# jamtrott/spmv-cache-trace

Measured on AMD Instinct MI355X. Metric: spmv_csr_gflops, higher is better.
Workload: dtype f64

## Files before the change

### spmv-cache-trace_amd/csrc/csr_runs.hpp

```cpp
#pragma once

#include "csr_wavetile.hpp"

namespace spmv {

constexpr int kRunChunkRows = 128;
constexpr int kRunWaves = 4;
constexpr int kRunLen = 5;
constexpr int kRunSlot = kRunLen * 128;

struct RunPattern {
    int rel[kRunLen];
};

__device__ __forceinline__ int4 scalar_load_i4(const int4 * p)
{
    typedef const v4i __attribute__((address_space(4))) * const_ptr;
    const v4i v = *reinterpret_cast<const_ptr>(reinterpret_cast<uintptr_t>(p));
    return make_int4(v[0], v[1], v[2], v[3]);
}

template <bool NT>
__device__ __forceinline__ void run_values_lds(const unsigned (&lds)[kRunLen], const double * ak, const unsigned (&o)[kRunLen])
{
    unsigned keep;
#define SPMV_RUN_DMA5(NTS)                                                                                                     \
    "s_nop 4\n\ts_mov_b32 %0, m0\n\t"                                                                                          \
    "s_mov_b32 m0, %1\n\ts_nop 0\n\tglobal_load_lds_dwordx4 %6, %11" NTS "\n\t"                                                \
    "s_mov_b32 m0, %2\n\ts_nop 0\n\tglobal_load_lds_dwordx4 %7, %11" NTS "\n\t"                                                \
    "s_mov_b32 m0, %3\n\ts_nop 0\n\tglobal_load_lds_dwordx4 %8, %11" NTS "\n\t"                                                \
    "s_mov_b32 m0, %4\n\ts_nop 0\n\tglobal_load_lds_dwordx4 %9, %11" NTS "\n\t"                                                \
    "s_mov_b32 m0, %5\n\ts_nop 0\n\tglobal_load_lds_dwordx4 %10, %11" NTS "\n\t"                                               \
    "s_mov_b32 m0, %0"
    if (NT)
        asm volatile(SPMV_RUN_DMA5(" nt") : "=&s"(keep) : "s"(lds[0]), "s"(lds[1]), "s"(lds[2]), "s"(lds[3]), "s"(lds[4]), "v"(o[0]),
                     "v"(o[1]), "v"(o[2]), "v"(o[3]), "v"(o[4]), "s"(ak) : "memory");
    else
        asm volatile(SPMV_RUN_DMA5("") : "=&s"(keep) : "s"(lds[0]), "s"(lds[1]), "s"(lds[2]), "s"(lds[3]), "s"(lds[4]), "v"(o[0]),
                     "v"(o[1]), "v"(o[2]), "v"(o[3]), "v"(o[4]), "s"(ak) : "memory");
#undef SPMV_RUN_DMA5
}

#define SPMV_RUN_ISSUE(LAST)                                                                                                   \
    "s_nop 4\n\t"                                                                                                              \
    "global_load_dwordx4 %0, %7, %8 nt\n\t"                                                                                    \
    "global_load_dwordx4 %1, %9, %14\n\t"                                                                                      \
    "global_load_dwordx4 %2, %10, %14\n\t"                                                                                     \
    "global_load_dwordx4 %3, %11, %14\n\t"                                                                                     \
    "global_load_dwordx4 %4, %12, %14\n\t"                                                                                     \
    "global_load_dwordx4 %5, %13, %14\n\t" LAST " %6, %15, %16\n\t"                                                            \
    "s_waitcnt vmcnt(0)"
__device__ __forceinline__ void run_issue_full(v2d_a8 & yv, v2d_a8 (&xv)[kRunLen], double & last, unsigned yo, const double * yb,
                                               const unsigned (&xo)[kRunLen], const double * x, unsigned lo, const double * ak)
{
    asm volatile(SPMV_RUN_ISSUE("global_load_dwordx2")
                 : "=&v"(yv), "=&v"(xv[0]), "=&v"(xv[1]), "=&v"(xv[2]), "=&v"(xv[3]), "=&v"(xv[4]), "=&v"(last)
                 : "v"(yo), "s"(yb), "v"(xo[0]), "v"(xo[1]), "v"(xo[2]), "v"(xo[3]), "v"(xo[4]), "s"(x), "v"(lo), "s"(ak)
                 : "memory");
}
__device__ __forceinline__ void run_issue_masked(v2d_a8 & yv, v2d_a8 (&xv)[kRunLen], unsigned & m2, unsigned yo, const double * yb,
                                                 const unsigned (&xo)[kRunLen], const double * x, unsigned mo, const uint8_t * mk)
{
    asm volatile(SPMV_RUN_ISSUE("global_load_ushort")
                 : "=&v"(yv), "=&v"(xv[0]), "=&v"(xv[1]), "=&v"(xv[2]), "=&v"(xv[3]), "=&v"(xv[4]), "=&v"(m2)
                 : "v"(yo), "s"(yb), "v"(xo[0]), "v"(xo[1]), "v"(xo[2]), "v"(xo[3]), "v"(xo[4]), "s"(x), "v"(mo), "s"(mk)
                 : "memory");
}
#undef SPMV_RUN_ISSUE

template <bool DENSE, bool NT>
__global__ __launch_bounds__(256) void csr_runs_kernel(int nchunks, int rows, int cols, const int4 * __restrict__ chunks,
                                                       const uint8_t * __restrict__ masks, RunPattern pat, const double * __restrict__ a,
                                                       const double * __restrict__ x, const double * y_in, double * y)
{
    __shared__ __attribute__((aligned(16))) double slots[kRunWaves][kRunSlot];
    const int wave = __builtin_amdgcn_readfirstlane((int) threadIdx.x >> 6);
    const int lane = (int) __lane_id();
    const int c = (int) blockIdx.x * kRunWaves + wave;
    asm volatile("" ::"s"(nchunks), "s"(rows), "s"(cols), "s"(chunks), "s"(masks), "s"(pat.rel[0]), "s"(pat.rel[1]), "s"(pat.rel[2]),
                 "s"(pat.rel[3]), "s"(pat.rel[4]), "s"(a), "s"(x), "s"(y_in), "s"(y));
    if (c >= nchunks)
        return;
    const double * slot = slots[wave];
    const unsigned lds = __builtin_amdgcn_readfirstlane((unsigned) reinterpret_cast<uintptr_t>((const __attribute__((address_space(3))) double *) slot));
    const int4 d = scalar_load_i4(chunks + c);
    const int row0 = DENSE ? c * kRunChunkRows : d.x;
    const int n = DENSE ? min(kRunChunkRows, rows - row0) : (d.z & 0xFF);
    const int e0 = d.y, entries = d.z >> 8, mslot = d.w;
    const int base = min(2 * lane, n - 2);
    const int kb = e0 & ~1, lead = e0 & 1;
    const int lastpair = ((e0 + entries - 1) & ~1) - kb;
    unsigned ldsi[kRunLen], vo[kRunLen];
#pragma unroll
    for (int i = 0; i < kRunLen; ++i) {
        ldsi[i] = lds + 1024u * i;
        vo[i] = 8u * (unsigned) min(128 * i + 2 * lane, lastpair);
    }
    int cx[kRunLen];
    unsigned xo[kRunLen];
#pragma unroll
    for (int p = 0; p < kRunLen; ++p) {
        cx[p] = row0 + base + pat.rel[p];
        xo[p] = 8u * (unsigned) min(max(cx[p], 0), cols - 2);
    }
    const double * ak = a + kb;
    run_values_lds<NT>(ldsi, ak, vo);
    v2d_a8 yv, xl[kRunLen];
    double zA = 0.0, zB = 0.0;
    if (mslot < 0) {
        double last;
        run_issue_full(yv, xl, last, 8u * (unsigned) base, y_in + row0, xo, x, 8u * (unsigned) (lead + entries - 1), ak);
        const double * v = slot + lead + base * kRunLen;
        const double vlast = base == n - 2 ? last : slot[min(lead + base * kRunLen + 2 * kRunLen - 1, kRunSlot - 1)];
#pragma unroll
        for (int p = 0; p < kRunLen; ++p) {
            zA += v[p] * xl[p].x;
            zB += (p == kRunLen - 1 ? vlast : v[kRunLen + p]) * xl[p].y;
        }
    } else {
        unsigned m2;
        run_issue_masked(yv, xl, m2, 8u * (unsigned) base, y_in + row0, xo, x, 2u * (unsigned) lane, masks + (size_t) mslot * kRunChunkRows);
        v2d_a8 xv[kRunLen];
#pragma unroll
        for (int p = 0; p < kRunLen; ++p)
            xv[p] = v2d_a8{cx[p] > cols - 2 ? xl[p].y : xl[p].x, cx[p] < 0 ? xl[p].x : xl[p].y};
        const unsigned m0 = m2 & 0xFFu, m1 = (m2 >> 8) & 0xFFu;
        const int cnt = __builtin_popcount(m0) + __builtin_popcount(m1);
        const int before = wave_inclusive_scan(cnt) - cnt;
        const bool own_pair = 2 * lane <= n - 2;
        const unsigned mA = own_pair ? m0 : 0u, mB = own_pair ? m1 : m0;
        int kA = lead + before, kB = lead + before + (own_pair ? __builtin_popcount(m0) : 0);
        double vA[kRunLen], vB[kRunLen];
#pragma unroll
        for (int p = 0; p < kRunLen; ++p) {
            vA[p] = slot[min(kA, kRunSlot - 1)];
            vB[p] = slot[min(kB, kRunSlot - 1)];
            kA += (mA >> p) & 1u;
            kB += (mB >> p) & 1u;
        }
        asm volatile("" : "+v"(vA[0]), "+v"(vA[1]), "+v"(vA[2]), "+v"(vA[3]), "+v"(vA[4]), "+v"(vB[0]), "+v"(vB[1]), "+v"(vB[2]), "+v"(vB[3]),
                     "+v"(vB[4]));
#pragma unroll
        for (int p = 0; p < kRunLen; ++p) {
            if ((mA >> p) & 1u)
                zA += vA[p] * xv[p].x;
            if ((mB >> p) & 1u)
                zB += vB[p] * xv[p].y;
        }
    }
    if (2 * lane <= n - 2) {
        const v2d_a8 out = {yv.x + zA, yv.y + zB};
        __builtin_nontemporal_store(out, reinterpret_cast<v2d_a8 *>(y + row0 + base));
    } else if (2 * lane == n - 1) {
        __builtin_nontemporal_store(yv.y + zB, y + row0 + base + 1);
    }
}

}
```

### spmv-cache-trace_amd/csrc/internal.hpp

```cpp
#pragma once

#include "spmv_hip_plan.h"
#include "spmv_hip_symmetric.h"
#include "spmv_hip_multivec.h"
#include "spmv_hip_transpose.h"
#include "spmv_hip_f32values.h"
#include "spmv_hip_compact.h"

#include <hip/hip_runtime.h>
#include <rccl/rccl.h>

#include <atomic>
#include <cstdint>
#include <string>
#include <vector>

#include "spmv_kernels.hpp"
#include "csr_segwin.hpp"

namespace spmvi {

int fail(int code, const char * what);
int fail_hip(hipError_t e, const char * call);
int check_csr_row_ptr(int32_t rows, int32_t cols, const int32_t * row_ptr);
// ... 47 lines not shown
    int long_blocks = 0;
    int32_t * d_blk_row = nullptr;
    int4 * d_tiles = nullptr;
    int ntiles = 0;
    int tile = 0;
    uint16_t * d_col16 = nullptr;
    const int32_t * compressed_from = nullptr;
    int narrow_tiles = 0;
    int shifted_tiles = 0;
    int xwin_tiles = 0;
    int longest_tile_row = 0;
    int spread_tiles = 0;
    spmv_hip_plan * inner = nullptr;
    int32_t * d_vrow_ptr = nullptr;
    int32_t * d_pcol = nullptr;
    double * d_pval = nullptr;
    const int32_t * panels_from_col = nullptr;
    const double * panels_from_val = nullptr;
    spmv::PanelInfo pinfo{};
    int panel_blocks = 0;
    int2 * d_blocks = nullptr;
    int nblocks16 = 0;
    int blockwin_tiles = 0;
    int32_t * d_rest_tiles = nullptr;
    int nrest_tiles = 0;
    int4 * d_run_chunks = nullptr;
    uint8_t * d_run_masks = nullptr;
    int32_t * d_run_rest = nullptr;
    int nrun_chunks = 0, nrun_rest = 0, run_len = 0, run_tiles = 0, run_masked_chunks = 0;
    long long run_entries = 0;
    spmv::RunPattern run_pattern{};
    bool run_dense = false;
    bool run_nt = false;
    int32_t * d_group_tiles = nullptr, * d_group_rest = nullptr;
    int ngroup_tiles = 0, ngroup_rest = 0;
    spmv::SegWinBlock * d_segblocks = nullptr;
    int nsegblocks = 0, seg_tiles_per_block = 0, segwin_tiles = 0, segwin_slots = 0;
    int32_t * d_patterns = nullptr;
    int npatterns = 0;
    int uniform_tiles = 0;
    int split_rows = 0;
    bool balanced = false;
    int32_t * d_colh = nullptr;
    int32_t * d_hub_column = nullptr;
    double * d_hubx = nullptr;
    int nhubs = 0, hub_threshold = 0;
    long long hub_entries = 0;
    int multi_window_tiles = 0;
    int block_hint = 0;
    int block_offset = 0;
    bool block_skewed = false;
    int hints_tried = 0;
    bool hint_from_bits = false;
    int colshare_tiles = 0;
    long long colshare_entries = 0;
    int block_candidate = 0;
    const uint32_t * group_bits = nullptr;
    int block_cuts = 0;
    int break_rows = 0;
    int block_tiles = 0;
    long long block_entries = 0;
    int stencil_mask_tiles = 0;
    long long stencil_mask_entries = 0;
    int masked_block_tiles = 0;
    long long masked_block_entries = 0;
    size_t meta_bytes = 0;
// ... 112 lines not shown
```

### spmv-cache-trace_amd/csrc/launch.hip

```cpp
#include "internal.hpp"
#ifdef SPMV_HIP_EXPERIMENTS
#include "csr_pipe.hpp"
#include <cstdlib>
#endif

#include <algorithm>

using namespace spmvi;

namespace {

template <int LPR>
void launch_vector(const spmv_hip_plan * pl, const int32_t * p, const int32_t * j, const double * a,
                   const double * x, double * y, hipStream_t s)
{
    hipLaunchKernelGGL((spmv::csr_vector_kernel<LPR, kBlock>), dim3(pl->workgroups), dim3(kBlock), 0, s,
                       pl->rows, p, j, a, x, y);
}

}

extern "C" {

int spmv_hip_csr_spmv(const spmv_hip_plan * pl, const int32_t * p, const int32_t * j,
                      const double * a, const double * x, double * y, void * stream)
{
    return spmv_hip_csr_spmv_out(pl, p, j, a, x, y, y, stream);
}

static int csr_spmv_launch(const spmv_hip_plan * pl, const int32_t * p, const int32_t * j, const double * a,
                           const double * x, const double * y_in, double * y, void * stream, const spmv::PeerY * peers, int * fused);

int spmv_hip_csr_spmv_out(const spmv_hip_plan * pl, const int32_t * p, const int32_t * j, const double * a,
                          const double * x, const double * y_in, double * y, void * stream)
{
    return csr_spmv_launch(pl, p, j, a, x, y_in, y, stream, nullptr, nullptr);
}

int spmv_hip_peer_push(const double * d_src, double * const * d_dst, int ndst, int64_t n, void * stream);

int spmv_hip_csr_spmv_out_peers(const spmv_hip_plan * pl, const int32_t * p, const int32_t * j, const double * a,
                                const double * x, const double * y_in, double * y, double * const * peer_y, int npeers,
                                int * fused_out, void * stream)
// ... 148 lines not shown
                                       pl->d_col16, a, x, y_in, y, pl->cols);
                    HIP_TRY(hipGetLastError());
                    return SPMV_HIP_OK;
                }
            }
#endif
            const int4 * vi_tiles = pl->d_tiles_vi ? pl->d_tiles_vi : pl->d_tiles;
            const int vi_ntiles = pl->d_tiles_vi ? pl->ntiles_vi : pl->ntiles;
            const unsigned vi_groups = (unsigned) ((vi_ntiles + 3) / 4);
            const bool all_blockwin = c16 && (pl->d_blocks || pl->d_segblocks) && pl->blockwin_tiles == pl->ntiles;
            const bool rest_forwards = peers && c16 && x32 && pl->d_segblocks && pl->split_rows == 0 && pl->tile == 512 && !xcd
                && (pl->blockwin_tiles == pl->ntiles || (pl->d_rest_tiles && pl->nrest_tiles > 0));
            if (all_blockwin) {
            } else if (rest_forwards) {
                hipLaunchKernelGGL((spmv::csr_wavetile_kernel<512, true, true, false, 0, 0, false, false, true, true>), dim3((unsigned) ((pl->nrest_tiles + 3) / 4)),
                                   dim3(256), 0, s, pl->nrest_tiles, pl->d_tiles, p, j, pl->d_col16, a, x, y_in, y, pl->nnz, pl->cols, exact, pl->d_patterns,
                                   spmv::PanelInfo{}, (const uint8_t *) nullptr, (const double *) nullptr, 0, *peers, pl->d_rest_tiles);
            } else if (c16 && (pl->d_blocks || pl->d_segblocks) && pl->d_rest_tiles && pl->nrest_tiles > 0 && pl->tile == 512 && !xcd) {
                const dim3 grid((unsigned) ((pl->nrest_tiles + 3) / 4));
                if (x32)
                    hipLaunchKernelGGL((spmv::csr_wavetile_kernel<512, true, true, false, 0, 0, false, false, false, true>), grid, dim3(256), 0, s,
                                       pl->nrest_tiles, pl->d_tiles, p, j, pl->d_col16, a, x, y_in, y, pl->nnz, pl->cols, exact, pl->d_patterns,
                                       spmv::PanelInfo{}, (const uint8_t *) nullptr, (const double *) nullptr, 0, spmv::PeerY{}, pl->d_rest_tiles);
                else
                    hipLaunchKernelGGL((spmv::csr_wavetile_kernel<512, true, false, false, 0, 0, false, false, false, true>), grid, dim3(256), 0, s,
                                       pl->nrest_tiles, pl->d_tiles, p, j, pl->d_col16, a, x, y_in, y, pl->nnz, pl->cols, exact, pl->d_patterns,
                                       spmv::PanelInfo{}, (const uint8_t *) nullptr, (const double *) nullptr, 0, spmv::PeerY{}, pl->d_rest_tiles);
            } else if (pl->d_run_chunks && pl->run_len == 5 && c16 && x32 && !xcd && !peers && !pl->d_group_tiles && !(pl->nvalues > 0 && pl->values_from == a)
                       && spmvi::aligned16(a)
#ifdef SPMV_HIP_EXPERIMENTS
                       && !abl
#endif
            ) {
                const dim3 grid((unsigned) ((pl->nrun_chunks + spmv::kRunWaves - 1) / spmv::kRunWaves));
                auto runs = pl->run_dense ? (pl->run_nt ? spmv::csr_runs_kernel<true, true> : spmv::csr_runs_kernel<true, false>)
                                          : (pl->run_nt ? spmv::csr_runs_kernel<false, true> : spmv::csr_runs_kernel<false, false>);
                hipLaunchKernelGGL(runs, grid, dim3(256), 0, s, pl->nrun_chunks, pl->rows, pl->cols, pl->d_run_chunks, pl->d_run_masks,
                                   pl->run_pattern, a, x, y_in, y);
                if (pl->nrun_rest > 0)
                    hipLaunchKernelGGL((spmv::csr_wavetile_kernel<512, true, true, false, 0, 0, false, false, false, true>), dim3((unsigned) ((pl->nrun_rest + 3) / 4)),
                                       dim3(256), 0, s, pl->nrun_rest, pl->d_tiles, p, j, pl->d_col16, a, x, y_in, y, pl->nnz, pl->cols, exact, pl->d_patterns,
                                       spmv::PanelInfo{}, (const uint8_t *) nullptr, (const double *) nullptr, 0, spmv::PeerY{}, pl->d_run_rest);
            } else
#ifdef SPMV_HIP_EXPERIMENTS
            if (pl->d_group_tiles && c16 && x32 && !xcd && !exact_order && pl->tile == 512 && (!peers || pl->split_rows == 0)) {
                const dim3 grid((unsigned) ((pl->ngroup_tiles + 3) / 4)), rest((unsigned) ((pl->ngroup_rest + 3) / 4));
                if (peers) {
                    hipLaunchKernelGGL((spmv::csr_rowgroup_kernel<true>), grid, dim3(256), 0, s, pl->ngroup_tiles, pl->d_group_tiles, pl->d_tiles, a, x, y_in,
                                       y, pl->cols, pl->d_patterns, *peers);
                    if (pl->ngroup_rest > 0)
                        hipLaunchKernelGGL((spmv::csr_wavetile_kernel<512, true, true, false, 0, 256, false, false, true, true>), rest, dim3(256), 0, s,
                                           pl->ngroup_rest, pl->d_tiles, p, j, pl->d_col16, a, x, y_in, y, pl->nnz, pl->cols, exact, pl->d_patterns,
                                           spmv::PanelInfo{}, (const uint8_t *) nullptr, (const double *) nullptr, 0, *peers, pl->d_group_rest);
                    *fused = 1;
                } else {
                    hipLaunchKernelGGL((spmv::csr_rowgroup_kernel<false>), grid, dim3(256), 0, s, pl->ngroup_tiles, pl->d_group_tiles, pl->d_tiles, a, x, y_in,
                                       y, pl->cols, pl->d_patterns);
                    if (pl->ngroup_rest > 0)
                        hipLaunchKernelGGL((spmv::csr_wavetile_kernel<512, true, true, false, 0, 256, false, false, false, true>), rest, dim3(256), 0, s,
                                           pl->ngroup_rest, pl->d_tiles, p, j, pl->d_col16, a, x, y_in, y, pl->nnz, pl->cols, exact, pl->d_patterns,
                                           spmv::PanelInfo{}, (const uint8_t *) nullptr, (const double *) nullptr, 0, spmv::PeerY{}, pl->d_group_rest);
                }
            } else
#endif
            if (!(pl->flags & SPMV_HIP_FLAG_NO_X_WINDOW) && (!exact_order || pl->longest_tile_row <= 32) && c16 && x32
                && pl->tile == 512 && !xcd && 2 * (long long) pl->xwin_tiles > pl->ntiles
                && !(pl->nvalues > 0 && pl->values_from == a) ) {
                if (peers && pl->split_rows == 0 && !pl->d_blocks && !pl->d_segblocks) {
                    hipLaunchKernelGGL((spmv::csr_wavetile_kernel<512, true, true, false, 0, 256, false, false, true>), dim3(pl->workgroups), dim3(256), 0, s,
                                       pl->ntiles, pl->d_tiles, p, j, pl->d_col16, a, x, y_in, y, pl->nnz, pl->cols, exact, pl->d_patterns, spmv::PanelInfo{},
                                       (const uint8_t *) nullptr, (const double *) nullptr, 0, *peers);
// ... 202 lines not shown
```

### spmv-cache-trace_amd/csrc/plan_csr.hip

```cpp
#include "internal.hpp"

#include <algorithm>
#include <cstdlib>
#include <cstring>
#include <new>
#include <system_error>
#include <thread>
#include <unordered_map>
#include <utility>

using namespace spmvi;

namespace {

constexpr size_t kStripedInts = (size_t) spmv::kCountStripes * spmv::kCountWidth;

template <typename T>
hipError_t read_striped(const T * d_counters, T * out, int n, hipStream_t s)
{
    T host[kStripedInts];
    hipError_t e = hipMemcpyAsync(host, d_counters, sizeof(host), hipMemcpyDeviceToHost, s);
    if (e == hipSuccess)
        e = hipStreamSynchronize(s);
    for (int i = 0; i < n; ++i) {
// ... 86 lines not shown
}

int verify_plan(const spmv_hip_plan * pl, const int32_t * d_column_index, hipStream_t s)
{
    if (!pl->d_col16 || pl->compressed_from != d_column_index)
        return SPMV_HIP_OK;
    unsigned long long sum = 0;
    int rc = device_column_checksum(d_column_index, pl->nnz, &sum, s);
    if (rc != SPMV_HIP_OK)
        return rc;
    if (sum != pl->column_checksum)
        return fail(SPMV_HIP_ERR_STATE, "the column array at this address is not the one the plan was compressed from "
                                        "(contents changed): make a new plan");
    return SPMV_HIP_OK;
}

static __global__ void run_gather_u16(const uint16_t * __restrict__ j16, const int32_t * __restrict__ idx, uint16_t * __restrict__ out, int n)
{
    const int i = (int) (blockIdx.x * blockDim.x + threadIdx.x);
    if (i < n)
        out[i] = j16[idx[i]];
}

void drop_stencil_runs(spmv_hip_plan * pl)
{
    for (void * q : {(void *) pl->d_run_chunks, (void *) pl->d_run_rest, (void *) pl->d_run_masks})
        if (q)
            (void) hipFree(q);
    pl->d_run_chunks = nullptr;
    pl->d_run_rest = nullptr;
    pl->d_run_masks = nullptr;
    pl->nrun_chunks = pl->nrun_rest = pl->run_len = pl->run_tiles = pl->run_masked_chunks = 0;
    pl->run_entries = 0;
    pl->run_dense = pl->run_nt = false;
}

static int build_stencil_runs(spmv_hip_plan * pl, const std::vector<int4> & d, bool compressed)
{
    drop_stencil_runs(pl);
    const bool exact_order = (pl->flags & SPMV_HIP_FLAG_EXACT_ORDER) != 0;
    const bool xwin_launch = !(pl->flags & SPMV_HIP_FLAG_NO_X_WINDOW) && (!exact_order || pl->longest_tile_row <= 32)
        && 2 * (long long) pl->xwin_tiles > pl->ntiles;
    if ((pl->flags & (SPMV_HIP_FLAG_NO_STENCIL_RUNS | SPMV_HIP_FLAG_XCD_REMAP)) || !compressed || pl->nvalues > 0 || pl->balanced
        || pl->inner || pl->d_blocks || pl->d_segblocks || pl->tile != 512 || pl->npatterns == 0 || pl->cols >= (1 << 29) || xwin_launch
        || pl->algorithm != SPMV_HIP_CSR_WAVETILE || pl->ntiles == 0 || pl->cols < 2)
        return SPMV_HIP_OK;
    bool align = true, masked = true, early = false, nt = true;
#ifdef SPMV_HIP_EXPERIMENTS
    if (const char * v = std::getenv("SPMV_HIP_RUNS_ALIGN")) align = std::atoi(v) != 0;
    if (const char * v = std::getenv("SPMV_HIP_RUNS_MASKED")) masked = std::atoi(v) != 0;
    if (const char * v = std::getenv("SPMV_HIP_RUNS_EARLY")) early = std::atoi(v) != 0;
    if (const char * v = std::getenv("SPMV_HIP_RUNS_NT")) nt = std::atoi(v) != 0;
#endif
    constexpr int L = spmv::kRunLen;
    const int ntiles = pl->ntiles;
    auto values_len = [&](int w) -> int {
        const int4 t = d[(size_t) w];
        const int meta = t.z;
        const int k0 = t.y, k1 = d[(size_t) w + 1].y;
        const int need = spmv::kTileMetaFast | spmv::kTileMetaShifted | spmv::kTileMetaUniform | spmv::kTileMetaPattern;
        if ((t.x & spmv::kTileFlagPartial) || k1 <= k0 || (meta & need) != need || ((meta >> spmv::kTileMetaLanesShift) & 7) != 0
            || (meta & (spmv::kTileMetaBlockWin | spmv::kTileMetaBlock3)) || spmv::is_masked_stencil_tile(meta) || k1 - (k0 & ~3) > 512)
            return 0;
        return meta & 0xFFFF;
    };
    auto narrow_tile = [&](int w) -> bool {
        const int4 t = d[(size_t) w];
        const int meta = t.z;
        const int k0 = t.y, k1 = d[(size_t) w + 1].y;
        const int need = spmv::kTileMetaFast | spmv::kTileMetaNarrow | spmv::kTileMetaUniform;
        const int nrows = (d[(size_t) w + 1].x & ~spmv::kTileFlagPartial) - t.x;
        return !(t.x & spmv::kTileFlagPartial) && k1 > k0 && (meta & need) == need && ((meta >> spmv::kTileMetaLanesShift) & 7) == 0
            && !(meta & (spmv::kTileMetaShifted | spmv::kTileMetaPattern | spmv::kTileMetaBlockWin | spmv::kTileMetaBlock3))
            && (meta & 0xFFFF) >= 1 && (meta & 0xFFFF) <= L && nrows >= 1 && nrows <= spmv::kRunChunkRows
            && (long long) nrows * (meta & 0xFFFF) == (long long) (k1 - k0) && k1 - (k0 & ~3) <= 512;
    };
    auto masked_tile = [&](int w) -> bool {
        const int4 t = d[(size_t) w];
        return !(t.x & spmv::kTileFlagPartial) && d[(size_t) w + 1].y > t.y && (t.z & spmv::kTileMetaFast) && spmv::is_masked_stencil_tile(t.z)
            && !(t.z & (spmv::kTileMetaBlockWin | spmv::kTileMetaBlock3));
    };
    std::vector<long long> per_pattern((size_t) pl->npatterns, 0);
    for (int w = 0; w < ntiles; ++w)
        if (values_len(w) == L && d[(size_t) w].w >= 0 && d[(size_t) w].w < pl->npatterns)
            per_pattern[(size_t) d[(size_t) w].w] += (long long) d[(size_t) w + 1].y - d[(size_t) w].y;
// ... 167 lines not shown
            c = stop;
        }
        if (e != d[(size_t) q].y)
            return SPMV_HIP_OK;
        r = end;
        w = q - 1;
    }
    if (chunks.empty() || 2 * entries <= (long long) pl->nnz)
        return SPMV_HIP_OK;
    std::sort(rest.begin(), rest.end());
    bool dense = early && (long long) chunks.size() == ((long long) pl->rows + spmv::kRunChunkRows - 1) / spmv::kRunChunkRows;
    for (size_t c = 0; c < chunks.size() && dense; ++c)
        dense = chunks[c].x == (int) c * spmv::kRunChunkRows && (chunks[c].z & 0xFF) == std::min(spmv::kRunChunkRows, pl->rows - chunks[c].x);
    HIP_TRY(hipMalloc((void **) &pl->d_run_chunks, chunks.size() * sizeof(int4)));
    HIP_TRY(hipMemcpy(pl->d_run_chunks, chunks.data(), chunks.size() * sizeof(int4), hipMemcpyHostToDevice));
    if (!cmasks.empty()) {
        HIP_TRY(hipMalloc((void **) &pl->d_run_masks, cmasks.size()));
        HIP_TRY(hipMemcpy(pl->d_run_masks, cmasks.data(), cmasks.size(), hipMemcpyHostToDevice));
    }
    pl->nrun_chunks = (int) chunks.size();
    pl->nrun_rest = (int) rest.size();
    pl->run_masked_chunks = (int) (cmasks.size() / spmv::kRunChunkRows);
    if (!rest.empty()) {
        rest.resize((rest.size() + 3) & ~(size_t) 3, rest.back());
        HIP_TRY(hipMalloc((void **) &pl->d_run_rest, rest.size() * sizeof(int32_t)));
        HIP_TRY(hipMemcpy(pl->d_run_rest, rest.data(), rest.size() * sizeof(int32_t), hipMemcpyHostToDevice));
    }
    pl->run_len = L;
    pl->run_tiles = tiles;
    pl->run_entries = entries;
    pl->run_pattern = rp;
    pl->run_dense = dense;
    pl->run_nt = nt;
    return SPMV_HIP_OK;
}

int plan_account(spmv_hip_plan * pl, bool compressed)
{
    const long long algorithmic = 12LL * pl->nnz + 4LL * (pl->rows + 1LL) + 16LL * pl->rows + 8LL * pl->cols;
    pl->streamed_bytes = algorithmic;
    pl->shifted_entries = pl->narrow_entries = pl->uniform_rows = 0;
    drop_stencil_runs(pl);
    if (pl->algorithm != SPMV_HIP_CSR_WAVETILE || pl->ntiles == 0)
        return SPMV_HIP_OK;
    const bool vi_tiles = pl->nvalues > 0 && pl->d_tiles_vi;
    const int ntiles = vi_tiles ? pl->ntiles_vi : pl->ntiles;
    std::vector<int4> d((size_t) ntiles + 1);
    HIP_TRY(hipMemcpy(d.data(), vi_tiles ? pl->d_tiles_vi : pl->d_tiles, d.size() * sizeof(int4), hipMemcpyDeviceToHost));
    long long bytes = 8LL * pl->cols;
    for (int w = 0; w < ntiles; ++w) {
        const long long entries = (long long) d[(size_t) w + 1].y - d[(size_t) w].y;
        const long long rows = (long long) (d[(size_t) w + 1].x & 0x7FFFFFFF) - (d[(size_t) w].x & 0x7FFFFFFF);
        const int meta = d[(size_t) w].z;
        const bool stream_tile = !(d[(size_t) w].x & 0x80000000) && entries > 0 && (meta & spmv::kTileMetaFast);
        const bool shifted = compressed && stream_tile && (meta & spmv::kTileMetaShifted);
        const bool narrow = compressed && stream_tile && (meta & spmv::kTileMetaNarrow);
        const bool uniform = stream_tile && (meta & spmv::kTileMetaUniform);
        const bool block3 = compressed && stream_tile && (meta & spmv::kTileMetaBlock3) && !(meta & spmv::kTileMetaBlockWin) && pl->nvalues == 0
            && !(pl->flags & SPMV_HIP_FLAG_EXACT_ORDER);
        if (compressed && stream_tile && spmv::is_masked_stencil_tile(meta)) {
            pl->shifted_entries += entries;
            bytes += (pl->nvalues > 0 ? 1 : 8) * entries + 2 * rows + 16 + 16 * rows;
            continue;
        }
        if (block3 && (meta & spmv::kTileMetaGroupRows)) {
            pl->narrow_entries += entries;
// ... 1687 lines not shown
        return SPMV_HIP_OK;
    return plan_account(pl, pl->d_col16 != nullptr);
}

int spmv_hip_plan_csr_refresh_values(spmv_hip_plan * pl, const int32_t * d_row_ptr, const int32_t * d_column_index,
                                     const double * d_value, void * stream)
{
    if (!pl)
        return fail(SPMV_HIP_ERR_INVALID, "plan is null");
    if (pl->nvalues > 0 || pl->d_vidx) {
        int rc = spmv_hip_plan_csr_index_values(pl, d_value, stream);
        if (rc != SPMV_HIP_OK)
            return rc;
    }
    if (!pl->inner)
        return SPMV_HIP_OK;
    if (!d_row_ptr || !d_column_index || !d_value)
        return fail(SPMV_HIP_ERR_INVALID, "null device pointer");
    if (d_column_index != pl->panels_from_col)
        return fail(SPMV_HIP_ERR_STATE, "the column panels were made from another column array");
    hipStream_t s = static_cast<hipStream_t>(stream);
    const unsigned grid = (unsigned) ((pl->rows + 255) / 256);
    hipLaunchKernelGGL(spmv::csr_panel_scatter_kernel, dim3(grid), dim3(256), 0, s, pl->rows, (pl->cols + 7) / 8, d_row_ptr,
                       d_column_index, d_value, pl->d_vrow_ptr, pl->d_pcol, pl->d_pval);
    HIP_TRY(hipGetLastError());
    pl->panels_from_val = d_value;
    return SPMV_HIP_OK;
}

int spmv_hip_plan_info(const spmv_hip_plan * pl, int64_t * out, int n)
{
    if (!pl || !out || n < 0)
        return fail(SPMV_HIP_ERR_INVALID, "plan/out null");
    const int64_t v[43] = {pl->algorithm, pl->lanes_per_row, pl->workgroups, pl->nblk,
                           pl->long_blocks, pl->rows, pl->nnz, (int64_t) pl->meta_bytes, pl->narrow_tiles,
                           pl->uniform_tiles, pl->shifted_tiles, pl->xwin_tiles, pl->blockwin_tiles,
                           pl->inner ? pl->inner->ntiles : 0, pl->streamed_bytes, pl->shifted_entries,
                           pl->narrow_entries, pl->uniform_rows, pl->inner ? 1 : 0, pl->balanced ? 1 : 0, pl->nvalues,
                           pl->segwin_tiles, pl->segwin_slots, pl->nvalues > 0 ? pl->value_row_tiles : 0,
                           pl->nvalues > 0 && pl->d_tiles_vi ? pl->ntiles_vi : 0, pl->nvalues > 0 ? 0 : pl->block_tiles,
                           pl->nvalues > 0 ? 0 : pl->block_entries, pl->nhubs, pl->hub_entries, pl->multi_window_tiles,
                           pl->ngroup_tiles, pl->nvalues > 0 ? 0 : pl->masked_block_tiles, pl->nvalues > 0 ? 0 : pl->masked_block_entries,
                           pl->stencil_mask_tiles, pl->stencil_mask_entries,
                           pl->nvalues > 0 ? 0 : pl->colshare_tiles, pl->nvalues > 0 ? 0 : pl->colshare_entries,
                           pl->colshare_tiles > 0 ? pl->block_hint : 0, pl->nrun_chunks, pl->run_tiles, pl->run_entries,
                           pl->run_masked_chunks, pl->nrun_chunks > 0 ? pl->nrun_rest : 0};
    for (int i = 0; i < n && i < 43; ++i)
        out[i] = v[i];
    return SPMV_HIP_OK;
}

}
```

### spmv-cache-trace_amd/python/spmv_amd/capi.py

```python
import ctypes as C
import os

import numpy as np

PKG_ROOT = os.path.dirname(os.path.dirname(os.path.dirname(os.path.abspath(__file__))))
LIB_PATH = os.path.join(PKG_ROOT, "libspmv_hip.so")
EXPERIMENTS_LIB_PATH = os.path.join(PKG_ROOT, "libspmv_hip_experiments.so")
if os.environ.get("SPMV_HIP_EXPERIMENTS") == "1":
    LIB_PATH = EXPERIMENTS_LIB_PATH
elif os.environ.get("SPMV_HIP_EXPERIMENTS", "").endswith(".so"):
    LIB_PATH = os.path.abspath(os.environ["SPMV_HIP_EXPERIMENTS"])
HEADER_PATH = os.path.join(os.path.dirname(PKG_ROOT), "include", "spmv_hip.h")
HEADER_PATHS = [HEADER_PATH] + [os.path.join(os.path.dirname(PKG_ROOT), "include", n)
                                for n in ("spmv_hip_tuning.h", "spmv_hip_plan.h", "spmv_hip_symmetric.h", "spmv_hip_multivec.h",
                                          "spmv_hip_transpose.h", "spmv_hip_f32values.h", "spmv_hip_compact.h")]

OK = 0
ERR_INVALID, ERR_NO_DEVICE, ERR_HIP, ERR_ALLOC, ERR_STATE, ERR_OVERFLOW, ERR_ALIGN = -1, -2, -3, -4, -5, -6, -7
CSR_AUTO, CSR_SCALAR, CSR_VECTOR, CSR_ADAPTIVE, CSR_WAVETILE = 0, 1, 2, 3, 4
FLAG_XCD_REMAP, FLAG_EXACT_ORDER, FLAG_BIG_TILE, FLAG_NO_INDEX_COMPRESSION, FLAG_COO_KEEP_ORDER, FLAG_READ_ROW_PTR, FLAG_ROWS64, FLAG_ROWS128, FLAG_ELL_COLUMN_MAJOR = 0x1, 0x2, 0x8, 0x10, 0x20, 0x40, 0x80, 0x100, 0x200
FLAG_NO_SHIFTED_TILES = 0x400
FLAG_PIPELINE_GATHER = 0x4
FLAG_NO_X_WINDOW = 0x800
FLAG_NO_COLUMN_PANELS = 0x1000
# ... 336 lines not shown
        check(self.lib.spmv_hip_last_run_times(self.h, C.byref(k), C.byref(g)))
        return k.value, g.value

    def info(self):
        out = np.zeros(20, dtype=np.int64)
        check(self.lib.spmv_hip_ctx_info(self.h, out, 20))
        keys = ["format", "rows", "cols", "stored", "algorithm", "lanes_per_row", "workgroups",
                "row_blocks", "long_blocks", "device_bytes", "narrow_tiles", "shifted_tiles", "xwin_tiles",
                "blockwin_tiles", "panel_tiles", "streamed_bytes", "devices", "ell_path", "rccl_ranks", "pipelined"]
        return dict(zip(keys, out.tolist()))


class CsrPlan:

    def __init__(self, rows, cols, host_row_ptr, algorithm=CSR_AUTO, lanes_per_row=0, flags=0):
        self.lib = load()
        h = _vp()
        check(self.lib.spmv_hip_plan_csr(C.byref(h), rows, cols, _i32(host_row_ptr), algorithm,
                                         lanes_per_row, flags))
        self.h = h

    def close(self):
        if self.h:
            self.lib.spmv_hip_plan_destroy(self.h)
            self.h = None

    def __del__(self):
        try:
            self.close()
        except Exception:
            pass

    def info(self):
        out = np.zeros(43, dtype=np.int64)
        check(self.lib.spmv_hip_plan_info(self.h, out, 43))
        keys = ["algorithm", "lanes_per_row", "workgroups", "row_blocks", "long_blocks", "rows",
                "nnz", "meta_bytes", "narrow_tiles", "uniform_tiles", "shifted_tiles", "xwin_tiles", "blockwin_tiles", "panel_tiles",
                "streamed_bytes", "shifted_entries", "narrow_entries", "uniform_rows", "value_snapshot", "balanced", "indexed_values",
                "segwin_tiles", "segwin_slots", "value_row_tiles", "dictionary_launch_tiles", "block_tiles", "block_entries", "hub_columns", "hub_entries", "multi_window_tiles", "row_group_tiles",
                "masked_block_tiles", "masked_block_entries", "stencil_mask_tiles", "stencil_mask_entries",
                "group_tiles", "group_entries", "group_rows", "run_chunks", "run_tiles", "run_entries",
                "run_masked_chunks", "run_rest_tiles"]
        return dict(zip(keys, out.tolist()))

    def confirm_blocks(self, d_row_ptr, d_col, host_row_ptr=None, stream=0):
        hp = None if host_row_ptr is None else np.ascontiguousarray(host_row_ptr, dtype=np.int32)
        check(self.lib.spmv_hip_plan_csr_confirm_blocks(self.h, d_row_ptr, d_col, None if hp is None else hp.ctypes.data, stream))

    def compress(self, d_col, stream=0):
        check(self.lib.spmv_hip_plan_csr_compress(self.h, d_col, stream))

    def repack(self, d_row_ptr, d_col, d_val, stream=0):
        check(self.lib.spmv_hip_plan_csr_repack(self.h, d_row_ptr, d_col, d_val, stream))

    def spmv(self, d_row_ptr, d_col, d_val, d_x, d_y, stream=0):
        check(self.lib.spmv_hip_csr_spmv(self.h, d_row_ptr, d_col, d_val, d_x, d_y, stream))

    def spmv_out(self, d_row_ptr, d_col, d_val, d_x, d_y_in, d_y_out, stream=0):
        check(self.lib.spmv_hip_csr_spmv_out(self.h, d_row_ptr, d_col, d_val, d_x, d_y_in, d_y_out, stream))

    def verify(self, d_col, stream=0):
        check(self.lib.spmv_hip_plan_verify(self.h, d_col, stream))

    def index_values(self, d_val, stream=0):
        check(self.lib.spmv_hip_plan_csr_index_values(self.h, d_val, stream))

    def refresh_values(self, d_row_ptr, d_col, d_val, stream=0):
        check(self.lib.spmv_hip_plan_csr_refresh_values(self.h, d_row_ptr, d_col, d_val, stream))


def csr_triangle(rows, row_ptr, col):
    row_ptr, col = _i32(row_ptr), _i32(col)
    if len(row_ptr) < rows + 1:
        raise ValueError("row_ptr needs rows + 1 entries")
    if len(col) == 0:
# ... 375 lines not shown
```

Measured before the change: 1106.

## Alternate run-kernel sweep direction across launches and make y nontemporal hints configurable

The stencil-runs kernel now processes its chunks in mirrored order on every other launch, reversing groups of eight workgroups so the per-group placement stays the same. The aim is that the chunks a launch touches first are the ones the previous launch touched last, so their matrix and vector data may still sit in L2 or the last-level cache. Nontemporal loads of y_in are now on only when the combined vector size exceeds a threshold, and the y store hint becomes a template option. In non-experiment builds the dense-chunk kernel variant is no longer selected, and a new plan-info field reports the variant. The costs are a host-side atomic counter per launch and a grid padded to a multiple of eight, whose extra blocks return early.

```diff
diff --git a/spmv-cache-trace_amd/csrc/csr_runs.hpp b/spmv-cache-trace_amd/csrc/csr_runs.hpp
--- a/spmv-cache-trace_amd/csrc/csr_runs.hpp
+++ b/spmv-cache-trace_amd/csrc/csr_runs.hpp
@@ -11,6 +11,7 @@
 
 struct RunPattern {
     int rel[kRunLen];
+    int mirror;
 };
 
 __device__ __forceinline__ int4 scalar_load_i4(const int4 * p)
@@ -41,34 +42,48 @@
 #undef SPMV_RUN_DMA5
 }
 
-#define SPMV_RUN_ISSUE(LAST)                                                                                                   \
+#define SPMV_RUN_ISSUE(YNT, LAST)                                                                                                \
     "s_nop 4\n\t"                                                                                                              \
-    "global_load_dwordx4 %0, %7, %8 nt\n\t"                                                                                    \
+    "global_load_dwordx4 %0, %7, %8" YNT "\n\t"                                                                                 \
     "global_load_dwordx4 %1, %9, %14\n\t"                                                                                      \
     "global_load_dwordx4 %2, %10, %14\n\t"                                                                                     \
     "global_load_dwordx4 %3, %11, %14\n\t"                                                                                     \
     "global_load_dwordx4 %4, %12, %14\n\t"                                                                                     \
     "global_load_dwordx4 %5, %13, %14\n\t" LAST " %6, %15, %16\n\t"                                                            \
     "s_waitcnt vmcnt(0)"
+#define SPMV_RUN_ISSUE_FULL(YNT)                                                                                               \
+    asm volatile(SPMV_RUN_ISSUE(YNT, "global_load_dwordx2")                                                                    \
+                 : "=&v"(yv), "=&v"(xv[0]), "=&v"(xv[1]), "=&v"(xv[2]), "=&v"(xv[3]), "=&v"(xv[4]), "=&v"(last)                \
+                 : "v"(yo), "s"(yb), "v"(xo[0]), "v"(xo[1]), "v"(xo[2]), "v"(xo[3]), "v"(xo[4]), "s"(x), "v"(lo), "s"(ak)      \
+                 : "memory")
+#define SPMV_RUN_ISSUE_MASKED(YNT)                                                                                             \
+    asm volatile(SPMV_RUN_ISSUE(YNT, "global_load_ushort")                                                                     \
+                 : "=&v"(yv), "=&v"(xv[0]), "=&v"(xv[1]), "=&v"(xv[2]), "=&v"(xv[3]), "=&v"(xv[4]), "=&v"(m2)                  \
+                 : "v"(yo), "s"(yb), "v"(xo[0]), "v"(xo[1]), "v"(xo[2]), "v"(xo[3]), "v"(xo[4]), "s"(x), "v"(mo), "s"(mk)      \
+                 : "memory")
+template <bool YIN_NT>
 __device__ __forceinline__ void run_issue_full(v2d_a8 & yv, v2d_a8 (&xv)[kRunLen], double & last, unsigned yo, const double * yb,
                                                const unsigned (&xo)[kRunLen], const double * x, unsigned lo, const double * ak)
 {
-    asm volatile(SPMV_RUN_ISSUE("global_load_dwordx2")
-                 : "=&v"(yv), "=&v"(xv[0]), "=&v"(xv[1]), "=&v"(xv[2]), "=&v"(xv[3]), "=&v"(xv[4]), "=&v"(last)
-                 : "v"(yo), "s"(yb), "v"(xo[0]), "v"(xo[1]), "v"(xo[2]), "v"(xo[3]), "v"(xo[4]), "s"(x), "v"(lo), "s"(ak)
-                 : "memory");
+    if (YIN_NT)
+        SPMV_RUN_ISSUE_FULL(" nt");
+    else
+        SPMV_RUN_ISSUE_FULL("");
 }
+template <bool YIN_NT>
 __device__ __forceinline__ void run_issue_masked(v2d_a8 & yv, v2d_a8 (&xv)[kRunLen], unsigned & m2, unsigned yo, const double * yb,
                                                  const unsigned (&xo)[kRunLen], const double * x, unsigned mo, const uint8_t * mk)
 {
-    asm volatile(SPMV_RUN_ISSUE("global_load_ushort")
-                 : "=&v"(yv), "=&v"(xv[0]), "=&v"(xv[1]), "=&v"(xv[2]), "=&v"(xv[3]), "=&v"(xv[4]), "=&v"(m2)
-                 : "v"(yo), "s"(yb), "v"(xo[0]), "v"(xo[1]), "v"(xo[2]), "v"(xo[3]), "v"(xo[4]), "s"(x), "v"(mo), "s"(mk)
-                 : "memory");
+    if (YIN_NT)
+        SPMV_RUN_ISSUE_MASKED(" nt");
+    else
+        SPMV_RUN_ISSUE_MASKED("");
 }
+#undef SPMV_RUN_ISSUE_MASKED
+#undef SPMV_RUN_ISSUE_FULL
 #undef SPMV_RUN_ISSUE
 
-template <bool DENSE, bool NT>
+template <bool DENSE, bool NT, bool YIN_NT = true, bool YOUT_NT = true>
 __global__ __launch_bounds__(256) void csr_runs_kernel(int nchunks, int rows, int cols, const int4 * __restrict__ chunks,
                                                        const uint8_t * __restrict__ masks, RunPattern pat, const double * __restrict__ a,
                                                        const double * __restrict__ x, const double * y_in, double * y)
@@ -76,9 +91,10 @@
     __shared__ __attribute__((aligned(16))) double slots[kRunWaves][kRunSlot];
     const int wave = __builtin_amdgcn_readfirstlane((int) threadIdx.x >> 6);
     const int lane = (int) __lane_id();
-    const int c = (int) blockIdx.x * kRunWaves + wave;
     asm volatile("" ::"s"(nchunks), "s"(rows), "s"(cols), "s"(chunks), "s"(masks), "s"(pat.rel[0]), "s"(pat.rel[1]), "s"(pat.rel[2]),
-                 "s"(pat.rel[3]), "s"(pat.rel[4]), "s"(a), "s"(x), "s"(y_in), "s"(y));
+                 "s"(pat.rel[3]), "s"(pat.rel[4]), "s"(pat.mirror), "s"(a), "s"(x), "s"(y_in), "s"(y));
+    const int b = (int) blockIdx.x;
+    const int c = (pat.mirror ? ((pat.mirror - 1 - (b >> 3)) << 3) | (b & 7) : b) * kRunWaves + wave;
     if (c >= nchunks)
         return;
     const double * slot = slots[wave];
@@ -109,7 +125,7 @@
     double zA = 0.0, zB = 0.0;
     if (mslot < 0) {
         double last;
-        run_issue_full(yv, xl, last, 8u * (unsigned) base, y_in + row0, xo, x, 8u * (unsigned) (lead + entries - 1), ak);
+        run_issue_full<YIN_NT>(yv, xl, last, 8u * (unsigned) base, y_in + row0, xo, x, 8u * (unsigned) (lead + entries - 1), ak);
         const double * v = slot + lead + base * kRunLen;
         const double vlast = base == n - 2 ? last : slot[min(lead + base * kRunLen + 2 * kRunLen - 1, kRunSlot - 1)];
 #pragma unroll
@@ -119,7 +135,7 @@
         }
     } else {
         unsigned m2;
-        run_issue_masked(yv, xl, m2, 8u * (unsigned) base, y_in + row0, xo, x, 2u * (unsigned) lane, masks + (size_t) mslot * kRunChunkRows);
+        run_issue_masked<YIN_NT>(yv, xl, m2, 8u * (unsigned) base, y_in + row0, xo, x, 2u * (unsigned) lane, masks + (size_t) mslot * kRunChunkRows);
         v2d_a8 xv[kRunLen];
 #pragma unroll
         for (int p = 0; p < kRunLen; ++p)
@@ -150,9 +166,15 @@
     }
     if (2 * lane <= n - 2) {
         const v2d_a8 out = {yv.x + zA, yv.y + zB};
-        __builtin_nontemporal_store(out, reinterpret_cast<v2d_a8 *>(y + row0 + base));
+        if (YOUT_NT)
+            __builtin_nontemporal_store(out, reinterpret_cast<v2d_a8 *>(y + row0 + base));
+        else
+            *reinterpret_cast<v2d_a8 *>(y + row0 + base) = out;
     } else if (2 * lane == n - 1) {
-        __builtin_nontemporal_store(yv.y + zB, y + row0 + base + 1);
+        if (YOUT_NT)
+            __builtin_nontemporal_store(yv.y + zB, y + row0 + base + 1);
+        else
+            y[row0 + base + 1] = yv.y + zB;
     }
 }
 
diff --git a/spmv-cache-trace_amd/csrc/internal.hpp b/spmv-cache-trace_amd/csrc/internal.hpp
--- a/spmv-cache-trace_amd/csrc/internal.hpp
+++ b/spmv-cache-trace_amd/csrc/internal.hpp
@@ -103,6 +103,8 @@
     spmv::RunPattern run_pattern{};
     bool run_dense = false;
     bool run_nt = false;
+    bool run_yin_nt = true, run_yout_nt = true, run_sweep = false;
+    mutable std::atomic<unsigned> run_launches{0};
     int32_t * d_group_tiles = nullptr, * d_group_rest = nullptr;
     int ngroup_tiles = 0, ngroup_rest = 0;
     spmv::SegWinBlock * d_segblocks = nullptr;
diff --git a/spmv-cache-trace_amd/csrc/launch.hip b/spmv-cache-trace_amd/csrc/launch.hip
--- a/spmv-cache-trace_amd/csrc/launch.hip
+++ b/spmv-cache-trace_amd/csrc/launch.hip
@@ -9,6 +9,13 @@
 using namespace spmvi;
 
 namespace {
+
+template <bool DENSE, bool NT>
+static auto run_kernel(bool yin_nt, bool yout_nt) -> decltype(&spmv::csr_runs_kernel<DENSE, NT, true, true>)
+{
+    return yin_nt ? (yout_nt ? spmv::csr_runs_kernel<DENSE, NT, true, true> : spmv::csr_runs_kernel<DENSE, NT, true, false>)
+                  : (yout_nt ? spmv::csr_runs_kernel<DENSE, NT, false, true> : spmv::csr_runs_kernel<DENSE, NT, false, false>);
+}
 
 template <int LPR>
 void launch_vector(const spmv_hip_plan * pl, const int32_t * p, const int32_t * j, const double * a,
@@ -223,11 +230,18 @@
                        && !abl
 #endif
             ) {
-                const dim3 grid((unsigned) ((pl->nrun_chunks + spmv::kRunWaves - 1) / spmv::kRunWaves));
-                auto runs = pl->run_dense ? (pl->run_nt ? spmv::csr_runs_kernel<true, true> : spmv::csr_runs_kernel<true, false>)
-                                          : (pl->run_nt ? spmv::csr_runs_kernel<false, true> : spmv::csr_runs_kernel<false, false>);
-                hipLaunchKernelGGL(runs, grid, dim3(256), 0, s, pl->nrun_chunks, pl->rows, pl->cols, pl->d_run_chunks, pl->d_run_masks,
-                                   pl->run_pattern, a, x, y_in, y);
+                const int groups = ((pl->nrun_chunks + spmv::kRunWaves - 1) / spmv::kRunWaves + 7) / 8;
+                const dim3 grid((unsigned) groups * 8u);
+                spmv::RunPattern pat = pl->run_pattern;
+                pat.mirror = pl->run_sweep && (pl->run_launches.fetch_add(1u, std::memory_order_relaxed) & 1u) ? groups : 0;
+                auto runs = run_kernel<false, true>(pl->run_yin_nt, pl->run_yout_nt);
+#ifdef SPMV_HIP_EXPERIMENTS
+                if (pl->run_dense)
+                    runs = pl->run_nt ? run_kernel<true, true>(pl->run_yin_nt, pl->run_yout_nt) : run_kernel<true, false>(pl->run_yin_nt, pl->run_yout_nt);
+                else if (!pl->run_nt)
+                    runs = run_kernel<false, false>(pl->run_yin_nt, pl->run_yout_nt);
+#endif
+                hipLaunchKernelGGL(runs, grid, dim3(256), 0, s, pl->nrun_chunks, pl->rows, pl->cols, pl->d_run_chunks, pl->d_run_masks, pat, a, x, y_in, y);
                 if (pl->nrun_rest > 0)
                     hipLaunchKernelGGL((spmv::csr_wavetile_kernel<512, true, true, false, 0, 0, false, false, false, true>), dim3((unsigned) ((pl->nrun_rest + 3) / 4)),
                                        dim3(256), 0, s, pl->nrun_rest, pl->d_tiles, p, j, pl->d_col16, a, x, y_in, y, pl->nnz, pl->cols, exact, pl->d_patterns,
diff --git a/spmv-cache-trace_amd/csrc/plan_csr.hip b/spmv-cache-trace_amd/csrc/plan_csr.hip
--- a/spmv-cache-trace_amd/csrc/plan_csr.hip
+++ b/spmv-cache-trace_amd/csrc/plan_csr.hip
@@ -142,7 +142,8 @@
     pl->d_run_masks = nullptr;
     pl->nrun_chunks = pl->nrun_rest = pl->run_len = pl->run_tiles = pl->run_masked_chunks = 0;
     pl->run_entries = 0;
-    pl->run_dense = pl->run_nt = false;
+    pl->run_dense = pl->run_nt = pl->run_sweep = false;
+    pl->run_yin_nt = pl->run_yout_nt = true;
 }
 
 static int build_stencil_runs(spmv_hip_plan * pl, const std::vector<int4> & d, bool compressed)
@@ -156,11 +157,15 @@
         || pl->algorithm != SPMV_HIP_CSR_WAVETILE || pl->ntiles == 0 || pl->cols < 2)
         return SPMV_HIP_OK;
     bool align = true, masked = true, early = false, nt = true;
+    bool sweep = true, yin_nt = 8LL * ((long long) pl->rows + pl->cols) > (256LL << 20), yout_nt = true;
 #ifdef SPMV_HIP_EXPERIMENTS
     if (const char * v = std::getenv("SPMV_HIP_RUNS_ALIGN")) align = std::atoi(v) != 0;
     if (const char * v = std::getenv("SPMV_HIP_RUNS_MASKED")) masked = std::atoi(v) != 0;
     if (const char * v = std::getenv("SPMV_HIP_RUNS_EARLY")) early = std::atoi(v) != 0;
     if (const char * v = std::getenv("SPMV_HIP_RUNS_NT")) nt = std::atoi(v) != 0;
+    if (const char * v = std::getenv("SPMV_HIP_RUNS_SWEEP")) sweep = std::atoi(v) != 0;
+    if (const char * v = std::getenv("SPMV_HIP_RUNS_YIN_NT")) yin_nt = std::atoi(v) != 0;
+    if (const char * v = std::getenv("SPMV_HIP_RUNS_YOUT_NT")) yout_nt = std::atoi(v) != 0;
 #endif
     constexpr int L = spmv::kRunLen;
     const int ntiles = pl->ntiles;
@@ -394,6 +399,9 @@
     pl->run_pattern = rp;
     pl->run_dense = dense;
     pl->run_nt = nt;
+    pl->run_sweep = sweep;
+    pl->run_yin_nt = yin_nt;
+    pl->run_yout_nt = yout_nt;
     return SPMV_HIP_OK;
 }
 
@@ -2147,7 +2155,7 @@
 {
     if (!pl || !out || n < 0)
         return fail(SPMV_HIP_ERR_INVALID, "plan/out null");
-    const int64_t v[43] = {pl->algorithm, pl->lanes_per_row, pl->workgroups, pl->nblk,
+    const int64_t v[44] = {pl->algorithm, pl->lanes_per_row, pl->workgroups, pl->nblk,
                            pl->long_blocks, pl->rows, pl->nnz, (int64_t) pl->meta_bytes, pl->narrow_tiles,
                            pl->uniform_tiles, pl->shifted_tiles, pl->xwin_tiles, pl->blockwin_tiles,
                            pl->inner ? pl->inner->ntiles : 0, pl->streamed_bytes, pl->shifted_entries,
@@ -2159,8 +2167,9 @@
                            pl->stencil_mask_tiles, pl->stencil_mask_entries,
                            pl->nvalues > 0 ? 0 : pl->colshare_tiles, pl->nvalues > 0 ? 0 : pl->colshare_entries,
                            pl->colshare_tiles > 0 ? pl->block_hint : 0, pl->nrun_chunks, pl->run_tiles, pl->run_entries,
-                           pl->run_masked_chunks, pl->nrun_chunks > 0 ? pl->nrun_rest : 0};
-    for (int i = 0; i < n && i < 43; ++i)
+                           pl->run_masked_chunks, pl->nrun_chunks > 0 ? pl->nrun_rest : 0,
+                           pl->nrun_chunks > 0 ? 1 + (pl->run_sweep ? 4 : 0) : 0};
+    for (int i = 0; i < n && i < 44; ++i)
         out[i] = v[i];
     return SPMV_HIP_OK;
 }
diff --git a/spmv-cache-trace_amd/python/spmv_amd/capi.py b/spmv-cache-trace_amd/python/spmv_amd/capi.py
--- a/spmv-cache-trace_amd/python/spmv_amd/capi.py
+++ b/spmv-cache-trace_amd/python/spmv_amd/capi.py
@@ -392,15 +392,15 @@
             pass
 
     def info(self):
-        out = np.zeros(43, dtype=np.int64)
-        check(self.lib.spmv_hip_plan_info(self.h, out, 43))
+        out = np.zeros(44, dtype=np.int64)
+        check(self.lib.spmv_hip_plan_info(self.h, out, 44))
         keys = ["algorithm", "lanes_per_row", "workgroups", "row_blocks", "long_blocks", "rows",
                 "nnz", "meta_bytes", "narrow_tiles", "uniform_tiles", "shifted_tiles", "xwin_tiles", "blockwin_tiles", "panel_tiles",
                 "streamed_bytes", "shifted_entries", "narrow_entries", "uniform_rows", "value_snapshot", "balanced", "indexed_values",
                 "segwin_tiles", "segwin_slots", "value_row_tiles", "dictionary_launch_tiles", "block_tiles", "block_entries", "hub_columns", "hub_entries", "multi_window_tiles", "row_group_tiles",
                 "masked_block_tiles", "masked_block_entries", "stencil_mask_tiles", "stencil_mask_entries",
                 "group_tiles", "group_entries", "group_rows", "run_chunks", "run_tiles", "run_entries",
-                "run_masked_chunks", "run_rest_tiles"]
+                "run_masked_chunks", "run_rest_tiles", "run_variant"]
         return dict(zip(keys, out.tolist()))
 
     def confirm_blocks(self, d_row_ptr, d_col, host_row_ptr=None, stream=0):
```

Result: faster. 1166, median of 6 (+5.4%).
